# r-barnes/richdem

Hardware: NVIDIA H100
Metric: Priority-Flood fill + D8 flow accumulation throughput (higher is better)
Workload: dtype f32

## Files before the change

richdem_b200/csrc/fill.cu:

```cuda
#include "common.cuh"

#include <chrono>

namespace rdb {

namespace {

#ifndef RDB_TX
#define RDB_TX 64
#endif
#ifndef RDB_TY
#define RDB_TY 64
#endif
#ifndef RDB_FILL_THREADS
#define RDB_FILL_THREADS 128
#endif
#ifndef RDB_FILL_MIN_CTAS
#define RDB_FILL_MIN_CTAS 6
#endif
constexpr int TX = RDB_TX;
constexpr int TY = RDB_TY;
constexpr int BXN = TX / 4;
constexpr int BYN = TY / 4;
constexpr int PADL = 4;
constexpr int SP = TX + 2 * PADL;
constexpr int SROWS = TY + 2;
constexpr int FILL_THREADS = RDB_FILL_THREADS;
constexpr int FILL_MIN_CTAS = RDB_FILL_MIN_CTAS;
static_assert(BYN <= 16 && BXN * BYN <= 256 && TX % 4 == 0 && TY % 4 == 0, "tile shape");
constexpr uint32_t W_TILE_BYTES = SP * SROWS * 4;
constexpr uint32_t Z_TILE_BYTES = TX * TY * 4;

struct RoundCtl {
  int count;
  int take;
};

struct FillDev {
  RoundCtl ctl[3];
  RoundCtl proc[3];
  unsigned long long visits;
  unsigned long long iters;
  unsigned long long block_updates;
  unsigned long long warp_updates;
  unsigned long long idle_visits;
  unsigned long long iter_hist[8];
  int edge_changed;
  int zmin_ord, zmax_ord;
  unsigned long long deferred;
  unsigned long long live_rounds;
  float level, step, step_min, level_max;
  int target, ordered;
  int ndefer[3];
};

struct FillArgs {
  const float *Z;
  int zpitch, zox, zoy, zext;
  const float *coarse;
  int Wc, pool, yoff;
  int *staged;
  float *Wp;
  int pitch;
  int W, H;
  int tilesX, tilesY;
  int *list0, *list1;
  int *stamp;
  int *sides;
  int *keys;
  float level;
  int *plist;
  int use_proc;
  FillDev *dev;
  int round;
  int max_iters;
  int use_tma;
  int profile;
  int *dirty;
};

__device__ __forceinline__ uint32_t smem_u32(const void *p) {
  return (uint32_t)__cvta_generic_to_shared(p);
}
// ... 34 lines not shown

constexpr int NBLK = BXN * BYN;
constexpr int MKP = BXN + 2;
constexpr int NWARP = FILL_THREADS / 32;
constexpr int SEG = ((NBLK + NWARP - 1) / NWARP + 31) / 32 * 32;
enum : int { SIDE_N = 1, SIDE_S = 2, SIDE_W = 4, SIDE_E = 8, SIDE_NW = 16, SIDE_NE = 32, SIDE_SW = 64,
             SIDE_SE = 128, SIDE_FULL = 256 };

__host__ __device__ __forceinline__ int f2ord(float f) {
  int b;
  memcpy(&b, &f, 4);
  return b >= 0 ? b : (b ^ 0x7fffffff);
}
__host__ __device__ __forceinline__ float ord2f(int o) {
  const int b = o >= 0 ? o : (o ^ 0x7fffffff);
  float f;
  memcpy(&f, &b, 4);
  return f;
}
constexpr int ORD_POS_INF = 0x7f800000;

__device__ __forceinline__ void enqueue_tile(const FillArgs &a, RoundCtl *next, int *list_next, int t,
                                             int stampval, int side_bits, int key_ord) {
  atomicOr(&a.sides[(stampval & 1) * a.tilesX * a.tilesY + t], side_bits);
  atomicMin(&a.keys[(stampval & 1) * a.tilesX * a.tilesY + t], key_ord);
  if (atomicExch(&a.stamp[t], stampval) != stampval) {
    const int idx = atomicAdd(&next->count, 1);
    list_next[idx] = t;
  }
}

__device__ __forceinline__ float min3f(float a, float b, float c) { return fminf(fminf(a, b), c); }

template <int STEP, bool TOPO4 = false, bool STAGE = false>
__global__ void __launch_bounds__(FILL_THREADS, FILL_MIN_CTAS)
    fill_sweep_kernel(const __grid_constant__ CUtensorMap mapW, const __grid_constant__ CUtensorMap mapZ,
                      const FillArgs a) {
  __shared__ __align__(128) float sW[SROWS * SP];
  __shared__ __align__(128) float sZ[TY * TX];
  __shared__ __align__(8) unsigned long long mbar;
  __shared__ unsigned char sMark[MKP * (BYN + 2)];
  __shared__ unsigned char sList[2][NWARP][SEG];
  __shared__ __align__(16) int sCnt[2][NWARP];
  __shared__ int sTile;
  __shared__ int sFlags;
  __shared__ int sKey;
  __shared__ int sProf[2];
  __shared__ int sNbDone;

  const int tid = threadIdx.x;
  const int r = a.round;
  RoundCtl *cur = &a.dev->ctl[r % 3];
  RoundCtl *next = &a.dev->ctl[(r + 1) % 3];
  const int *list_cur = (r & 1) ? a.list1 : a.list0;
  int *list_next = (r & 1) ? a.list0 : a.list1;
  const int ntiles = a.tilesX * a.tilesY;
  if (a.use_proc) {
    cur = &a.dev->proc[r % 3];
    list_cur = a.plist;
  }
  const int n = cur->count;

  if (blockIdx.x == 0 && tid == 0) {
    RoundCtl *z = &a.dev->ctl[(r + 2) % 3];
    z->count = 0;
    z->take = 0;
    RoundCtl *zp = &a.dev->proc[(r + 1) % 3];
    zp->count = 0;
    zp->take = 0;
    if (n > 0) {
      atomicAdd(&a.dev->visits, (unsigned long long)n);
      a.dev->live_rounds++;
    }
  }
  if (n == 0) return;

  if (tid == 0) {
    mbar_init(&mbar, 1);
    asm volatile("fence.mbarrier_init.release.cluster;" ::: "memory");
  }
  uint32_t phase = 0;
  const int max_iters = a.max_iters;

  for (;;) {
    if (tid == 0) sTile = atomicAdd(&cur->take, 1);
    for (int k = tid; k < MKP * (BYN + 2); k += FILL_THREADS) sMark[k] = 0;
    __syncthreads();
    const int li = sTile;
    if (li >= n) break;
    const int t = list_cur[li];
    const int tyT = t / a.tilesX, txT = t - tyT * a.tilesX;
    const int x0 = txT * TX, y0 = tyT * TY;

    constexpr bool stage = STAGE;
    if (tid == 0) {
      sFlags = 0;
      sKey = ORD_POS_INF;
      sProf[0] = sProf[1] = 0;
      if (stage) {
        int nb = 0;
        for (int dy = -1; dy <= 1; dy++)
          for (int dx = -1; dx <= 1; dx++) {
            const int ty = tyT + dy, tx = txT + dx;
            if ((dx | dy) && ty >= 0 && ty < a.tilesY && tx >= 0 && tx < a.tilesX &&
                *reinterpret_cast<volatile int *>(&a.staged[ty * a.tilesX + tx]))
              nb |= 1 << ((dy + 1) * 3 + dx + 1);
          }
        __threadfence();
        sNbDone = nb;
      }
    }
    if (a.use_tma) {
      if (tid == 0) {
        fence_proxy_async();
        mbar_arrive_expect_tx(&mbar, (stage ? 0u : W_TILE_BYTES) + Z_TILE_BYTES);
        if (!stage) tma_load_2d(sW, &mapW, x0, y0, &mbar);
        tma_load_2d(sZ, &mapZ, x0 + a.zox, y0 + a.zoy, &mbar);
      }
    } else {
      if (!stage) {
        for (int k = tid; k < SROWS * (SP / 4); k += FILL_THREADS) {
          const int rr = k / (SP / 4), cc = k - rr * (SP / 4);
          reinterpret_cast<float4 *>(sW)[k] =
              __ldcg(reinterpret_cast<const float4 *>(a.Wp + (size_t)(y0 + rr) * a.pitch + x0) + cc);
        }
      }
      const float inf = __int_as_float(0x7f800000);
      for (int k = tid; k < TY * (TX / 4); k += FILL_THREADS) {
        const int rr = k / (TX / 4), cc = k - rr * (TX / 4);
        reinterpret_cast<float4 *>(sZ)[k] =
            a.zext && (y0 + rr >= a.H || x0 + 4 * cc >= a.W)
                ? make_float4(inf, inf, inf, inf)
                : __ldg(reinterpret_cast<const float4 *>(a.Z + (size_t)(y0 + a.zoy + rr) * a.zpitch + x0 + a.zox) + cc);
      }
    }
    int sides = a.sides[(r & 1) * ntiles + t];
    __syncthreads();
    if (tid == 0) {
      a.sides[(r & 1) * ntiles + t] = 0;
      a.keys[(r & 1) * ntiles + t] = ORD_POS_INF;
    }
    if (stage) {
      const float inf = __int_as_float(0x7f800000);
      const int nbdone = sNbDone;
      for (int k = tid; k < SROWS * (SP / 4); k += FILL_THREADS) {
        const int rr = k / (SP / 4), c4 = 4 * (k - rr * (SP / 4));
        const int dy = rr == 0 ? -1 : (rr == SROWS - 1 ? 1 : 0), dx = c4 < PADL ? -1 : (c4 >= PADL + TX ? 1 : 0);
        float4 v4;
        if ((nbdone >> ((dy + 1) * 3 + dx + 1)) & 1) {
          v4 = __ldcg(reinterpret_cast<const float4 *>(a.Wp + (size_t)(y0 + rr) * a.pitch + x0 + c4));
        } else {
          const int y = y0 + rr - 1, xb = x0 + c4 - PADL;
          float v[4] = {inf, inf, inf, inf};
          if (y >= 0 && y < a.H) {
            const float *crow = a.coarse + (size_t)((y + a.yoff) / a.pool) * a.Wc;
            const float *zrow = a.Z + (size_t)(y + a.zoy) * a.zpitch + a.zox;
            const bool brow = y == 0 || y == a.H - 1;
            const float c0 = (a.pool & 3) == 0 && xb >= 0 && xb < a.W ? __ldg(crow + xb / a.pool) : inf;
#pragma unroll
            for (int j = 0; j < 4; j++) {
              const int x = xb + j;
              if (x >= 0 && x < a.W)
                v[j] = brow || x == 0 || x == a.W - 1 ? __ldg(zrow + x) : (a.pool & 3) == 0 ? c0 : __ldg(crow + x / a.pool);
            }
          }
          v4 = make_float4(v[0], v[1], v[2], v[3]);
        }
        *reinterpret_cast<float4 *>(&sW[rr * SP + c4]) = v4;
      }
    }
#include "fill_relax_body.inc"

    if (f) {
      atomicOr(&sFlags, f);
      if (f & 0xFF) atomicMin(&sKey, f2ord(kmin));
    }
    __syncthreads();
    const int fl = sFlags;
    const int rowch = (fl >> 12) & 0xFFFF;
    const int rowout = stage ? (1 << BYN) - 1 : rowch;
    if (rowout) {
      for (int k = tid; k < TY * (TX / 4); k += FILL_THREADS) {
        const int rr = k / (TX / 4), cc = k % (TX / 4);
        if (rowout & (1 << (rr >> 2))) {
          const float4 val = *reinterpret_cast<const float4 *>(&sW[(rr + 1) * SP + PADL + 4 * cc]);
          __stcg(reinterpret_cast<float4 *>(a.Wp + (size_t)(y0 + 1 + rr) * a.pitch + (x0 + PADL)) + cc, val);
        }
      }
    }
    if (stage) {
      __syncthreads();
      if (tid == 0) {
        __threadfence();
        atomicExch(&a.staged[t], 1);
      }
    }
    if (rowch) {
      if (tid < 8) {
        const int sv = r + 1;
        const bool n_ok = tyT > 0, s_ok = tyT < a.tilesY - 1, w_ok = txT > 0, e_ok = txT < a.tilesX - 1;
        int nb = -1, bits = 0;
        switch (tid) {
          case 0: if ((fl & SIDE_N) && n_ok) { nb = t - a.tilesX; bits = SIDE_S; } break;
          case 1: if ((fl & SIDE_S) && s_ok) { nb = t + a.tilesX; bits = SIDE_N; } break;
          case 2: if ((fl & SIDE_W) && w_ok) { nb = t - 1; bits = SIDE_E; } break;
          case 3: if ((fl & SIDE_E) && e_ok) { nb = t + 1; bits = SIDE_W; } break;
          case 4: if ((fl & SIDE_NW) && n_ok && w_ok) { nb = t - a.tilesX - 1; bits = SIDE_SE; } break;
          case 5: if ((fl & SIDE_NE) && n_ok && e_ok) { nb = t - a.tilesX + 1; bits = SIDE_SW; } break;
          case 6: if ((fl & SIDE_SW) && s_ok && w_ok) { nb = t + a.tilesX - 1; bits = SIDE_NE; } break;
          default: if ((fl & SIDE_SE) && s_ok && e_ok) { nb = t + a.tilesX + 1; bits = SIDE_NW; } break;
        }
        if (nb >= 0) enqueue_tile(a, next, list_next, nb, sv, bits, sKey);
        if (tid == 0 && (fl & (3 << 9))) atomicOr(&a.dev->edge_changed, (fl >> 9) & 3);
        if (tid == 0 && a.dirty) a.dirty[t] = 1;
      }
    }
    if (tid == 0) {
      if (again) enqueue_tile(a, next, list_next, t, r + 1, SIDE_FULL, f2ord(-__int_as_float(0x7f800000)));
      atomicAdd(&a.dev->iters, (unsigned long long)iters);
      if (a.profile) {
        if (!rowch) atomicAdd(&a.dev->idle_visits, 1ull);
        atomicAdd(&a.dev->block_updates, (unsigned long long)sProf[0]);
        atomicAdd(&a.dev->warp_updates, (unsigned long long)sProf[1]);
        const int hb = iters <= 1 ? 0 : iters <= 2 ? 1 : iters <= 4 ? 2 : iters <= 8 ? 3 : iters <= 16 ? 4 : iters <= 32 ? 5 : iters <= 64 ? 6 : 7;
        atomicAdd(&a.dev->iter_hist[hb], 1ull);
      }
    }
  }
}

__global__ void __launch_bounds__(256) fill_admit_kernel(const FillArgs a) {
  const int r = a.round;
  const RoundCtl *cur = &a.dev->ctl[r % 3];
  RoundCtl *next = &a.dev->ctl[(r + 1) % 3];
  RoundCtl *proc = &a.dev->proc[r % 3];
  const int *list_cur = (r & 1) ? a.list1 : a.list0;
  int *list_next = (r & 1) ? a.list0 : a.list1;
  const int n = cur->count;
  const int ntiles = a.tilesX * a.tilesY;
  const float level = a.level;
  int nd = 0;
  for (int i = blockIdx.x * blockDim.x + threadIdx.x; i < n; i += gridDim.x * blockDim.x) {
    const int t = list_cur[i];
    const int kord = a.keys[(r & 1) * ntiles + t];
    if (ord2f(kord) <= level) {
      a.plist[atomicAdd(&proc->count, 1)] = t;
    } else {
      int bits = a.sides[(r & 1) * ntiles + t];
      if (bits == 0) bits = SIDE_FULL;
      a.sides[(r & 1) * ntiles + t] = 0;
      a.keys[(r & 1) * ntiles + t] = ORD_POS_INF;
      enqueue_tile(a, next, list_next, t, r + 1, bits, kord);
      nd++;
    }
  }
  for (int o = 16; o > 0; o >>= 1) nd += __shfl_xor_sync(0xffffffffu, nd, o);
  if ((threadIdx.x & 31) == 0 && nd) atomicAdd(&a.dev->ndefer[r % 3], nd);
}

// ... 660 lines not shown
    if (!still_active) first_run = false;
    live_rounds = (int64_t)hd->live_rounds;
    visits_seen = (int64_t)hd->visits;
    iters_seen = (int64_t)hd->iters;
    batch_edge = hd->edge_changed;
    return still_active;
  }
  int64_t iters_seen = 0;

  int run(int64_t max_rounds = 0) {
    Ctx &c = ctx();
    int64_t rounds_this_call = 0;
    int per_sync = (int)(c.params.fill_rounds_per_sync > 0 ? c.params.fill_rounds_per_sync : 16);
    if (max_rounds > 0 && max_rounds < per_sync) per_sync = (int)max_rounds;
    RDB_CK(cudaMemsetAsync(&dev.p->edge_changed, 0, sizeof(int), c.stream));
    for (;;) {
      launch_batch(per_sync);
      collect();
      rounds_this_call += per_sync;
      if (!still_active) break;
      if (max_rounds > 0 && rounds_this_call >= max_rounds) break;
    }
    const FillDev *hd = (const FillDev *)c.pinned;
    c.stats.fill_rounds = live_rounds;
    c.stats.fill_tile_visits = visits_seen;
    c.stats.fill_tile_iters = iters_seen;
    c.stats.fill_tile_cells = TX * TY;
    if (c.params.fill_profile) {
      fprintf(stderr, "[fill profile] deferred=%llu visits=%llu iters=%llu block_updates=%llu (%.1f%% of 256/iter) warp_updates=%llu (%.1f%% of 8/iter) idle_visits=%llu hist(1,2,3-4,5-8,9-16,17-32,33-64,65+)=",
              hd->deferred, hd->visits, hd->iters, hd->block_updates, 100.0 * hd->block_updates / (256.0 * hd->iters + 1),
              hd->warp_updates, 100.0 * hd->warp_updates / (8.0 * hd->iters + 1), hd->idle_visits);
      for (int k = 0; k < 8; k++) fprintf(stderr, "%llu ", hd->iter_hist[k]);
      fprintf(stderr, "\n");
    }
    return batch_edge | (still_active ? 4 : 0);
  }

  void track_dirty() {
    Ctx &c = ctx();
    const size_t nt = (size_t)tilesX * tilesY;
    dirty.alloc(nt);
    RDB_CK(cudaMemsetAsync(dirty.p, 0, nt * sizeof(int), c.stream));
  }
  void clear_dirty() {
    if (dirty.p) RDB_CK(cudaMemsetAsync(dirty.p, 0, (size_t)tilesX * tilesY * sizeof(int), ctx().stream));
  }
  void seed_from_flags(int *d_count = nullptr) {
    Ctx &c = ctx();
    const int nt = tilesX * tilesY;
    FillArgs a = make_args();
    a.round = round;
    fill_seed_flags_kernel<<<(nt + 255) / 256, 256, 0, c.stream>>>(a, tflag.p, nt, d_count);
    RDB_CK(cudaGetLastError());
    count_launch();
  }
  void clear_flags() {
    const size_t nt = (size_t)tilesX * tilesY;
    if (!tflag.p) tflag.alloc(nt);
    RDB_CK(cudaMemsetAsync(tflag.p, 0, nt * sizeof(int), ctx().stream));
  }
  void restrict_into(FillState &cs, int k) {
    Ctx &c = ctx();
    cs.clear_flags();
    const bool selective = dirty.p && TX % k == 0 && TY % k == 0;
    dim3 blk(256), grd((unsigned)((cs.W + 255) / 256), (unsigned)(cs.H < 4096 ? cs.H : 4096));
    fill_restrict_kernel<<<grd, blk, 0, c.stream>>>(Wp.p, pitch, W, H, cs.Wp.p, cs.pitch, cs.W, cs.H, k,
// ... 620 lines not shown
```

richdem_b200/csrc/accum.cu:

```cuda
#include "flowmet.cuh"

#include <cmath>
#include <cooperative_groups.h>
namespace cg = cooperative_groups;

namespace rdb {

namespace {

constexpr uint32_t kDepsMask = 0xFFu;
constexpr uint32_t kSrcFlag = 0x80000000u;
constexpr int kCodeSole = 32;
constexpr int kCodeSource = 64;
constexpr int kLaneChunk = 1024;

template <bool DINF>
__global__ void __launch_bounds__(256) flow_code_kernel(const float *__restrict__ dem, uint8_t *__restrict__ code,
                                                         float *__restrict__ rmaxArr, double *__restrict__ accum,
                                                         int W, int H, float nodata, int ones, int tfilter) {
  const size_t n = (size_t)W * H;
  const size_t i = (size_t)blockIdx.x * blockDim.x + threadIdx.x;
  if (i >= n) return;
  const int y = (int)(i / W), x = (int)(i - (size_t)y * W);
  int cd;
// ... 1402 lines not shown
    frontier[atomicAdd(fcount, 1)] = base_index + x;
  } else {
    row[x] = (left << 56) | val;
  }
}

constexpr int kFaT = 64;
constexpr int kFaCells = kFaT * kFaT;
constexpr int kFaSlots = 4 * kFaT;
constexpr unsigned long long kLkOne = 1ull << 32;

__device__ __forceinline__ int fa_side(int left) { return left < kFaT ? left : kFaT; }

__device__ __forceinline__ int fa_slot_of(int lx, int ly, int tw, int th) {
  if (ly == 0) return lx;
  if (ly == th - 1) return kFaT + lx;
  if (lx == 0) return 2 * kFaT + ly;
  if (lx == tw - 1) return 3 * kFaT + ly;
  return -1;
}

__device__ __forceinline__ bool fa_slot_cell(int s, int tw, int th, int &lx, int &ly) {
  const int k = s & (kFaT - 1), side = s / kFaT;
  if (side < 2) {
    lx = k;
    ly = side == 0 ? 0 : th - 1;
    return k < tw && (side == 0 || th > 1);
  }
  lx = side == 2 ? 0 : tw - 1;
  ly = k;
  return k > 0 && k < th - 1 && (side == 2 || tw > 1);
}

__device__ __forceinline__ void fa_tile_accumulate(const uint8_t *sCode, unsigned long long *sWord, uint16_t *sQueue,
                                                   int *sCount, int tw, int th) {
  const int t = threadIdx.x;
  for (int k = 0; k < kFaCells / 256; k++) {
    const int c = t + 256 * k, lx = c & (kFaT - 1), ly = c / kFaT;
    if (sCode[c] == kCodeNoData) continue;
    unsigned deps = 0;
#pragma unroll
    for (int n = 1; n <= 8; n++) {
      const int x = lx + d8dx(n), y = ly + d8dy(n);
      if (x >= 0 && y >= 0 && x < tw && y < th && (sCode[y * kFaT + x] & 15) == d8_inverse(n)) deps++;
    }
    if (deps) sWord[c] += (unsigned long long)deps << 56;
    else sQueue[atomicAdd(&sCount[0], 1)] = (uint16_t)c;
  }
  __syncthreads();
  const int nsrc = sCount[0];
  int cur = 0;
  unsigned long long acc = 0;
  bool walking = false;
  for (;;) {
    if (!walking) {
      const int i = atomicAdd(&sCount[1], 1);
      if (i >= nsrc) break;
      cur = sQueue[i];
      acc = sWord[cur];
      walking = true;
    }
    const int d = sCode[cur] & 15;
    const int x = (cur & (kFaT - 1)) + d8dx(d), y = cur / kFaT + d8dy(d);
    if (d == 0 || x < 0 || y < 0 || x >= tw || y >= th) {
      walking = false;
      continue;
    }
    const int r = y * kFaT + x;
    const unsigned long long old = atomicAdd(&sWord[r], acc - kPkOne);
    if ((old >> 56) != 1ull) {
      walking = false;
      continue;
    }
    acc = (old & kPkVal) + acc;
    cur = r;
  }
  __syncthreads();
}

constexpr int kFaRootExit = 0x8000, kFaRootEnd = 0x4000;

__global__ void __launch_bounds__(256) fa_tile_codes_kernel(const float *__restrict__ dem, uint8_t *__restrict__ code,
                                                             int *__restrict__ link, unsigned long long *__restrict__ lword,
                                                             unsigned *__restrict__ inflow, int W, int H, float nodata,
                                                             int tiles_x) {
  constexpr int kWin = kFaT + 2;
  static_assert(kFaCells * sizeof(uint16_t) <= kWin * kWin * sizeof(float), "the parent array lives in the DEM window");
  __shared__ __align__(16) float sDem[kWin * kWin];
  __shared__ __align__(16) uint8_t sCode[kFaCells];
  __shared__ unsigned sCount[kFaSlots];
  const int t = threadIdx.x, tile = blockIdx.x;
  sCount[t] = 0;
  const int bx = tile % tiles_x, by = tile / tiles_x;
  const int x0 = bx * kFaT, y0 = by * kFaT;
  const int tw = fa_side(W - x0), th = fa_side(H - y0);
  for (int i = t; i < kWin * kWin; i += 256) {
    const int wy = i / kWin, wx = i - wy * kWin;
    const int gy = y0 - 1 + wy, gx = x0 - 1 + wx;
    sDem[i] = (gy >= 0 && gy < H && gx >= 0 && gx < W) ? __ldg(dem + (size_t)gy * W + gx) : nodata;
  }
  __syncthreads();
  {
    const int lx = t & (kFaT - 1), ly0 = (t / kFaT) * (kFaT / 4);
    float a[3][3];
#pragma unroll
    for (int j = 1; j < 3; j++)
#pragma unroll
      for (int k = 0; k < 3; k++) a[j][k] = sDem[(ly0 + j - 1) * kWin + lx + k];
    for (int j = 0; j < kFaT / 4; j++) {
      const int ly = ly0 + j;
#pragma unroll
      for (int k = 0; k < 3; k++) {
        a[0][k] = a[1][k];
        a[1][k] = a[2][k];
        a[2][k] = sDem[(ly + 2) * kWin + lx + k];
      }
      const float e = a[1][1];
      const int gx = x0 + lx, gy = y0 + ly;
      int cd = 0;
      if (lx >= tw || ly >= th || e == nodata) {
        cd = kCodeNoData;
      } else if (!(gx == 0 || gy == 0 || gx == W - 1 || gy == H - 1)) {
        const float ne[9] = {0.f, a[1][0], a[0][0], a[0][1], a[0][2], a[1][2], a[2][2], a[2][1], a[2][0]};
        float lowest = fminf(e, 3.402823466e+38f);
#pragma unroll
        for (int n = 1; n <= 8; n++) {
          const float v = ne[n];
          if (v < lowest && v != nodata) {
            lowest = v;
            cd = n;
          }
        }
      }
      sCode[ly * kFaT + lx] = (uint8_t)cd;
    }
  }
  __syncthreads();
  reinterpret_cast<uint4 *>(code + (size_t)tile * kFaCells)[t] = reinterpret_cast<const uint4 *>(sCode)[t];
  uint16_t *sPar = reinterpret_cast<uint16_t *>(sDem);
  unsigned live = 0;
#pragma unroll
  for (int k = 0; k < kFaCells / 256; k++) {
    const int c = t + 256 * k, cd = sCode[c], d = cd & 15;
    int p = c | kFaRootEnd;
    if (cd != kCodeNoData && d != 0) {
      const int x = (c & (kFaT - 1)) + d8dx(d), y = c / kFaT + d8dy(d);
      if (x < 0 || y < 0 || x >= tw || y >= th) {
        p = c | kFaRootExit;
      } else {
        p = y * kFaT + x;
        live |= 1u << k;
      }
    }
    sPar[c] = (uint16_t)p;
  }
  while (__syncthreads_or(live)) {
#pragma unroll
    for (int k = 0; k < kFaCells / 256; k++) {
      if (live >> k & 1) {
        const int c = t + 256 * k, q = sPar[sPar[c]];
        sPar[c] = (uint16_t)q;
        if (q & (kFaRootExit | kFaRootEnd)) live &= ~(1u << k);
      }
    }
  }
#pragma unroll
  for (int k = 0; k < kFaCells / 256; k++) {
    const int r = sPar[t + 256 * k];
    if (r & kFaRootExit) atomicAdd(&sCount[fa_slot_of(r & (kFaT - 1), (r & (kFaCells - 1)) / kFaT, tw, th)], 1u);
  }
  __syncthreads();
  const size_t gs = (size_t)tile * kFaSlots + t;
  int lk = -1;
  unsigned long long out = 0;
  int lx, ly;
  if (fa_slot_cell(t, tw, th, lx, ly)) {
    const int c = ly * kFaT + lx, r = sPar[c];
    if (r == (c | kFaRootExit)) {
      const int d = sCode[c] & 15;
      const int gx = x0 + lx + d8dx(d), gy = y0 + ly + d8dy(d), rbx = gx / kFaT, rby = gy / kFaT;
      const int rs = fa_slot_of(gx - rbx * kFaT, gy - rby * kFaT, fa_side(W - rbx * kFaT), fa_side(H - rby * kFaT));
      lk = -2 - ((rby * tiles_x + rbx) * kFaSlots + rs);
      out = kLkOne | sCount[t];
    } else if (r & kFaRootExit) {
      const int e = r & (kFaCells - 1);
      lk = tile * kFaSlots + fa_slot_of(e & (kFaT - 1), e / kFaT, tw, th);
    }
  }
  link[gs] = lk;
  lword[gs] = out;
  inflow[gs] = 0;
}

__device__ __forceinline__ int fa_link_next(const int *link, int r) {
  const int l = link[r];
  return l <= -2 ? r : l;
}

__global__ void __launch_bounds__(256) fa_link_count_kernel(const int *__restrict__ link, unsigned long long *lword,
                                                             int nslots) {
  const int p = blockIdx.x * blockDim.x + threadIdx.x;
  if (p >= nslots) return;
  const int l = link[p];
  if (l > -2) return;
  const int q = fa_link_next(link, -2 - l);
  if (q >= 0) atomicAdd(&lword[q], kLkOne);
}

__global__ void __launch_bounds__(256) fa_link_walk_kernel(const int *__restrict__ link, unsigned long long *lword,
                                                            unsigned *inflow, int nslots) {
  const int p = blockIdx.x * blockDim.x + threadIdx.x;
  if (p >= nslots) return;
  int l = link[p];
  if (l > -2) return;
  const unsigned long long old = atomicAdd(&lword[p], 0ull - kLkOne);
  if ((old >> 32) != 1ull) return;
  unsigned long long acc = old & (kLkOne - 1);
  for (;;) {
    const int r = -2 - l;
    atomicAdd(&inflow[r], (unsigned)acc);
    const int q = fa_link_next(link, r);
    if (q < 0) break;
    const unsigned long long o = atomicAdd(&lword[q], acc - kLkOne);
    if ((o >> 32) != 1ull) break;
    acc = (o & (kLkOne - 1)) + acc;
    l = link[q];
  }
}

__global__ void __launch_bounds__(256) fa_tile_final_kernel(const uint8_t *__restrict__ code,
                                                             const unsigned *__restrict__ inflow, double *__restrict__ accum,
                                                             int W, int H, int tiles_x) {
  __shared__ __align__(16) unsigned long long sWord[kFaCells];
  __shared__ __align__(16) uint8_t sCode[kFaCells];
  __shared__ uint16_t sQueue[kFaCells];
  __shared__ int sCount[2];
  const int t = threadIdx.x, tile = blockIdx.x;
  const int bx = tile % tiles_x, by = tile / tiles_x;
  const int x0 = bx * kFaT, y0 = by * kFaT;
  const int tw = fa_side(W - x0), th = fa_side(H - y0);
  if (t < 2) sCount[t] = 0;
  reinterpret_cast<uint4 *>(sCode)[t] = __ldg(reinterpret_cast<const uint4 *>(code + (size_t)tile * kFaCells) + t);
  for (int c = t; c < kFaCells; c += 256) sWord[c] = 1;
  __syncthreads();
  int lx, ly;
  if (fa_slot_cell(t, tw, th, lx, ly)) sWord[ly * kFaT + lx] += __ldg(inflow + (size_t)tile * kFaSlots + t);
  __syncthreads();
  fa_tile_accumulate(sCode, sWord, sQueue, sCount, tw, th);
  for (int c = t; c < kFaCells; c += 256) {
    const int cx = c & (kFaT - 1), cy = c / kFaT;
    if (cx < tw && cy < th)
      accum[(size_t)(y0 + cy) * W + x0 + cx] = sCode[c] == kCodeNoData ? -1.0 : (double)(sWord[c] & kPkVal);
  }
}

long long fa_tile_slots(int w, int h) {
  return (long long)((w + kFaT - 1) / kFaT) * ((h + kFaT - 1) / kFaT) * kFaSlots;
}

void fa_d8_tiles(const float *d_dem, double *d_accum, int w, int h, float nodata) {
  Ctx &c = ctx();
  const int tiles_x = (w + kFaT - 1) / kFaT;
  const long long nslots = fa_tile_slots(w, h);
  const unsigned ntiles = (unsigned)(nslots / kFaSlots);
  DevBuf<uint8_t> code((size_t)ntiles * kFaCells);
  DevBuf<int> link((size_t)nslots);
  DevBuf<unsigned long long> lword((size_t)nslots);
  DevBuf<unsigned> inflow((size_t)nslots);
  const unsigned sblocks = (unsigned)((nslots + 255) / 256);
  fa_tile_codes_kernel<<<ntiles, 256, 0, c.stream>>>(d_dem, code.p, link.p, lword.p, inflow.p, w, h, nodata, tiles_x);
  fa_link_count_kernel<<<sblocks, 256, 0, c.stream>>>(link.p, lword.p, (int)nslots);
  KernelTimer kt;
  fa_link_walk_kernel<<<sblocks, 256, 0, c.stream>>>(link.p, lword.p, inflow.p, (int)nslots);
  kt.stop_async();
  fa_tile_final_kernel<<<ntiles, 256, 0, c.stream>>>(code.p, inflow.p, d_accum, w, h, tiles_x);
  RDB_CK(cudaGetLastError());
  count_launch(4);
  RDB_CK(cudaStreamSynchronize(c.stream));
  c.stats.ms_main_kernel += kt.ms();
  c.stats.accum_rounds = 1;
}
}

void fa_fused_dev(const float *d_dem, double *d_accum, int w, int h, float nodata, bool ones, bool dinf) {
  Ctx &c = ctx();
  const size_t n = (size_t)w * h;
// ... 865 lines not shown
  FACC_TRY
  state->st.collect_frontier();
  int a = 0, b = 0;
  state->st.run(&a, &b);
  if (sent_top) *sent_top = a;
  if (sent_bottom) *sent_bottom = b;
  FACC_END
}

int rdb200_dev_facc_take_outflow(rdb200_facc_state *state, int32_t which, double *d_sum_row, int32_t *d_cnt_row) {
  FACC_TRY
  state->st.take_outflow(which, d_sum_row, d_cnt_row);
  RDB_CK(cudaStreamSynchronize(rdb::ctx().stream));
  FACC_END
}

int rdb200_dev_facc_apply_inflow(rdb200_facc_state *state, int32_t which, const double *d_sum_row,
                                 const int32_t *d_cnt_row) {
  FACC_TRY
  state->st.apply_inflow(which, d_sum_row, d_cnt_row);
  RDB_CK(cudaStreamSynchronize(rdb::ctx().stream));
  FACC_END
}

int rdb200_dev_facc_finish(rdb200_facc_state *state) {
  FACC_TRY
  if (state) {
    RDB_CK(cudaStreamSynchronize(rdb::ctx().stream));
    delete state;
  }
  FACC_END
}

}
```

richdem_b200/csrc/fill_relax_body.inc:

```
    if (sides == 0) sides = SIDE_FULL;
    const int lane = tid & 31, wrp = tid >> 5;
    {
      int cntw = 0;
#pragma unroll
      for (int q = 0; q < SEG / 32; q++) {
        const int b = wrp * SEG + 32 * q + lane;
        const int bx = b % BXN, by = b / BXN;
        bool on = (sides & SIDE_FULL) != 0;
        on |= (sides & SIDE_N) && by == 0;
        on |= (sides & SIDE_S) && by == BYN - 1;
        on |= (sides & SIDE_W) && bx == 0;
        on |= (sides & SIDE_E) && bx == BXN - 1;
        on |= (sides & SIDE_NW) && b == 0;
        on |= (sides & SIDE_NE) && b == BXN - 1;
        on |= (sides & SIDE_SW) && b == NBLK - BXN;
        on |= (sides & SIDE_SE) && b == NBLK - 1;
        on &= b < NBLK;
        const unsigned bal = __ballot_sync(0xffffffffu, on);
        if (on) sList[0][wrp][cntw + __popc(bal & ((1u << lane) - 1u))] = (unsigned char)b;
        cntw += __popc(bal);
      }
      if (lane == 0) sCnt[0][wrp] = cntw;
    }
    if (a.use_tma) {
      mbar_wait(&mbar, phase);
      phase ^= 1;
      if (a.zext && (x0 + TX > a.W || y0 + TY > a.H)) {
        for (int k = tid; k < TX * TY; k += FILL_THREADS) {
          const int rr = k / TX, cc = k - rr * TX;
          if (y0 + rr >= a.H || x0 + cc >= a.W) sZ[k] = __int_as_float(0x7f800000);
        }
      }
    }
    __syncthreads();

    int f = 0;
    float kmin = __int_as_float(0x7f800000);
    int iters = 0;
    int cl = 0;
    bool again = false;
    int segn[NWARP];
    int nlist = 0;
#pragma unroll
    for (int w2 = 0; w2 < NWARP; w2++) {
      segn[w2] = sCnt[0][w2];
      nlist += segn[w2];
    }
    while (nlist > 0) {
      for (int i = tid; i < nlist; i += FILL_THREADS) {
        int seg = 0, off = i;
#pragma unroll
        for (int w2 = 0; w2 < NWARP - 1; w2++) {
          if (seg == w2 && off >= segn[w2]) {
            off -= segn[w2];
            seg = w2 + 1;
          }
        }
        const int b = sList[cl][seg][off];
        const int bx = b % BXN, by = b / BXN;
        const int srow = 4 * by + 1, scol = 4 * bx + PADL;
        float v[6][6];
        float z[4][4];
        bool at_floor = true;
#pragma unroll
        for (int j = 0; j < 4; j++) {
          const float4 z4 = *reinterpret_cast<const float4 *>(&sZ[(4 * by + j) * TX + 4 * bx]);
          const float4 m4 = *reinterpret_cast<const float4 *>(&sW[(srow + j) * SP + scol]);
// ... 120 lines not shown
```

Measured before the change: 18250.

## Prefetch next tile index and issue TMA early in staged fill sweep

In the staged fill kernel, the next tile index is now claimed from the work queue right after relaxation and before the write-back and enqueue phase, which hides the atomic's latency. TMA loads are issued before the per-tile flag setup rather than after it. Division by the pooling factor uses a shift when the factor is a power of two. The change also adds optional per-phase clock profiling counters. Taking the next tile early changes the order in which tiles are claimed, and it adds a few extra atomics when profiling is on.

```diff
diff --git a/richdem_b200/csrc/fill.cu b/richdem_b200/csrc/fill.cu
--- a/richdem_b200/csrc/fill.cu
+++ b/richdem_b200/csrc/fill.cu
@@ -49,6 +49,7 @@
   int zmin_ord, zmax_ord;
   unsigned long long deferred;
   unsigned long long live_rounds;
+  unsigned long long st_visits, st_iters, st_block_updates, st_hist[8], st_clk[3];
   float level, step, step_min, level_max;
   int target, ordered;
   int ndefer[3];
@@ -149,6 +150,14 @@
 
 __device__ __forceinline__ float min3f(float a, float b, float c) { return fminf(fminf(a, b), c); }
 
+__device__ __forceinline__ unsigned long long prof_clock() {
+#ifdef RDB_EMU
+  return 0;
+#else
+  return clock64();
+#endif
+}
+
 template <int STEP, bool TOPO4 = false, bool STAGE = false>
 __global__ void __launch_bounds__(FILL_THREADS, FILL_MIN_CTAS)
     fill_sweep_kernel(const __grid_constant__ CUtensorMap mapW, const __grid_constant__ CUtensorMap mapZ,
@@ -163,6 +172,7 @@
   __shared__ int sFlags;
   __shared__ int sKey;
   __shared__ int sProf[2];
+  __shared__ unsigned long long sClk;
   __shared__ int sNbDone;
 
   const int tid = threadIdx.x;
@@ -198,18 +208,33 @@
   }
   uint32_t phase = 0;
   const int max_iters = a.max_iters;
-
+  auto prof_phase = [&](int k) {
+    const unsigned long long now = prof_clock();
+    if (k >= 0) atomicAdd(&a.dev->st_clk[k], now - sClk);
+    sClk = now;
+  };
+
+  if (STAGE && tid == 0) sTile = atomicAdd(&cur->take, 1);
   for (;;) {
-    if (tid == 0) sTile = atomicAdd(&cur->take, 1);
+    if (!STAGE && tid == 0) sTile = atomicAdd(&cur->take, 1);
     for (int k = tid; k < MKP * (BYN + 2); k += FILL_THREADS) sMark[k] = 0;
     __syncthreads();
     const int li = sTile;
     if (li >= n) break;
+    if constexpr (STAGE) {
+      if (a.profile && tid == 0) prof_phase(-1);
+    }
     const int t = list_cur[li];
     const int tyT = t / a.tilesX, txT = t - tyT * a.tilesX;
     const int x0 = txT * TX, y0 = tyT * TY;
 
     constexpr bool stage = STAGE;
+    if (a.use_tma && tid == 0) {
+      fence_proxy_async();
+      mbar_arrive_expect_tx(&mbar, (stage ? 0u : W_TILE_BYTES) + Z_TILE_BYTES);
+      if (!stage) tma_load_2d(sW, &mapW, x0, y0, &mbar);
+      tma_load_2d(sZ, &mapZ, x0 + a.zox, y0 + a.zoy, &mbar);
+    }
     if (tid == 0) {
       sFlags = 0;
       sKey = ORD_POS_INF;
@@ -227,14 +252,7 @@
         sNbDone = nb;
       }
     }
-    if (a.use_tma) {
-      if (tid == 0) {
-        fence_proxy_async();
-        mbar_arrive_expect_tx(&mbar, (stage ? 0u : W_TILE_BYTES) + Z_TILE_BYTES);
-        if (!stage) tma_load_2d(sW, &mapW, x0, y0, &mbar);
-        tma_load_2d(sZ, &mapZ, x0 + a.zox, y0 + a.zoy, &mbar);
-      }
-    } else {
+    if (!a.use_tma) {
       if (!stage) {
         for (int k = tid; k < SROWS * (SP / 4); k += FILL_THREADS) {
           const int rr = k / (SP / 4), cc = k - rr * (SP / 4);
@@ -260,6 +278,7 @@
     if (stage) {
       const float inf = __int_as_float(0x7f800000);
       const int nbdone = sNbDone;
+      const int psh = (a.pool & (a.pool - 1)) == 0 ? __ffs(a.pool) - 1 : -1;
       for (int k = tid; k < SROWS * (SP / 4); k += FILL_THREADS) {
         const int rr = k / (SP / 4), c4 = 4 * (k - rr * (SP / 4));
         const int dy = rr == 0 ? -1 : (rr == SROWS - 1 ? 1 : 0), dx = c4 < PADL ? -1 : (c4 >= PADL + TX ? 1 : 0);
@@ -270,15 +289,18 @@
           const int y = y0 + rr - 1, xb = x0 + c4 - PADL;
           float v[4] = {inf, inf, inf, inf};
           if (y >= 0 && y < a.H) {
-            const float *crow = a.coarse + (size_t)((y + a.yoff) / a.pool) * a.Wc;
+            const int cy = psh >= 0 ? (y + a.yoff) >> psh : (y + a.yoff) / a.pool;
+            const float *crow = a.coarse + (size_t)cy * a.Wc;
             const float *zrow = a.Z + (size_t)(y + a.zoy) * a.zpitch + a.zox;
             const bool brow = y == 0 || y == a.H - 1;
-            const float c0 = (a.pool & 3) == 0 && xb >= 0 && xb < a.W ? __ldg(crow + xb / a.pool) : inf;
+            const float c0 = (a.pool & 3) == 0 && xb >= 0 && xb < a.W ? __ldg(crow + (psh >= 0 ? xb >> psh : xb / a.pool)) : inf;
 #pragma unroll
             for (int j = 0; j < 4; j++) {
               const int x = xb + j;
               if (x >= 0 && x < a.W)
-                v[j] = brow || x == 0 || x == a.W - 1 ? __ldg(zrow + x) : (a.pool & 3) == 0 ? c0 : __ldg(crow + x / a.pool);
+                v[j] = brow || x == 0 || x == a.W - 1 ? __ldg(zrow + x)
+                       : (a.pool & 3) == 0            ? c0
+                                                      : __ldg(crow + (psh >= 0 ? x >> psh : x / a.pool));
             }
           }
           v4 = make_float4(v[0], v[1], v[2], v[3]);
@@ -286,7 +308,15 @@
         *reinterpret_cast<float4 *>(&sW[rr * SP + c4]) = v4;
       }
     }
+    if constexpr (STAGE) {
+      if (a.profile && tid == 0) prof_phase(0);
+    }
 #include "fill_relax_body.inc"
+    int next_li = 0;
+    if constexpr (STAGE) {
+      if (a.profile && tid == 0) prof_phase(1);
+      if (tid == 0) next_li = atomicAdd(&cur->take, 1);
+    }
 
     if (f) {
       atomicOr(&sFlags, f);
@@ -341,7 +371,15 @@
         atomicAdd(&a.dev->warp_updates, (unsigned long long)sProf[1]);
         const int hb = iters <= 1 ? 0 : iters <= 2 ? 1 : iters <= 4 ? 2 : iters <= 8 ? 3 : iters <= 16 ? 4 : iters <= 32 ? 5 : iters <= 64 ? 6 : 7;
         atomicAdd(&a.dev->iter_hist[hb], 1ull);
-      }
+        if constexpr (STAGE) {
+          atomicAdd(&a.dev->st_visits, 1ull);
+          atomicAdd(&a.dev->st_iters, (unsigned long long)iters);
+          atomicAdd(&a.dev->st_block_updates, (unsigned long long)sProf[0]);
+          atomicAdd(&a.dev->st_hist[hb], 1ull);
+          prof_phase(2);
+        }
+      }
+      if (STAGE) sTile = next_li;
     }
   }
 }
@@ -1068,6 +1106,16 @@
               hd->warp_updates, 100.0 * hd->warp_updates / (8.0 * hd->iters + 1), hd->idle_visits);
       for (int k = 0; k < 8; k++) fprintf(stderr, "%llu ", hd->iter_hist[k]);
       fprintf(stderr, "\n");
+      if (hd->st_visits) {
+        const double v = (double)hd->st_visits;
+        const double clk = (double)(hd->st_clk[0] + hd->st_clk[1] + hd->st_clk[2]);
+        fprintf(stderr, "[fill profile staged] w=%d h=%d visits=%llu passes/visit=%.2f block_updates/visit=%.1f "
+                        "hist(1,2,3-4,5-8,9-16,17-32,33-64,65+)=",
+                W, H, hd->st_visits, hd->st_iters / v, hd->st_block_updates / v);
+        for (int k = 0; k < 8; k++) fprintf(stderr, "%llu ", hd->st_hist[k]);
+        fprintf(stderr, "clk/visit=%.0f build=%.1f%% relax=%.1f%% write=%.1f%%\n", clk / v, 100.0 * hd->st_clk[0] / clk,
+                100.0 * hd->st_clk[1] / clk, 100.0 * hd->st_clk[2] / clk);
+      }
     }
     return batch_edge | (still_active ? 4 : 0);
   }
```

New measurement: 18380 (median of 6 runs). About the same (+0.7%).

## Pack tile accumulation into 32-bit words with donor counts from code pass

Applied to the files above, without the earlier changes.

The tile-final accumulation now uses 32-bit packed shared words (donor count, direction, local sum) and stores boundary inflow in a separate array that is carried along walks, replacing 64-bit words and the neighbour-scan dependency count. Donor counts are computed once in the codes kernel by atomically adding into the upper nibble of each code byte. Sources are enqueued with a warp prefix scan instead of per-cell atomics. The aim is to cut shared-memory footprint and setup work, at the cost of extra atomics and fences whenever inflow is carried. Optional clock64 phase probes are added behind a macro.

```diff
diff --git a/richdem_b200/csrc/accum.cu b/richdem_b200/csrc/accum.cu
--- a/richdem_b200/csrc/accum.cu
+++ b/richdem_b200/csrc/accum.cu
@@ -1458,47 +1458,70 @@
   return k > 0 && k < th - 1 && (side == 2 || tw > 1);
 }
 
-__device__ __forceinline__ void fa_tile_accumulate(const uint8_t *sCode, unsigned long long *sWord, uint16_t *sQueue,
-                                                   int *sCount, int tw, int th) {
-  const int t = threadIdx.x;
-  for (int k = 0; k < kFaCells / 256; k++) {
-    const int c = t + 256 * k, lx = c & (kFaT - 1), ly = c / kFaT;
-    if (sCode[c] == kCodeNoData) continue;
-    unsigned deps = 0;
-#pragma unroll
-    for (int n = 1; n <= 8; n++) {
-      const int x = lx + d8dx(n), y = ly + d8dy(n);
-      if (x >= 0 && y >= 0 && x < tw && y < th && (sCode[y * kFaT + x] & 15) == d8_inverse(n)) deps++;
-    }
-    if (deps) sWord[c] += (unsigned long long)deps << 56;
-    else sQueue[atomicAdd(&sCount[0], 1)] = (uint16_t)c;
-  }
-  __syncthreads();
-  const int nsrc = sCount[0];
-  int cur = 0;
-  unsigned long long acc = 0;
+#ifdef RDB_FA_PHASE_CLOCKS
+constexpr int kFaPhases = 8;
+__device__ unsigned long long g_fa_phase_clk[2 * kFaPhases];
+#define FA_PHASE_START() long long fa_clk = clock64()
+#define FA_PHASE_END(i)                                                    \
+  do {                                                                     \
+    __syncthreads();                                                       \
+    if (threadIdx.x == 0) {                                                \
+      const long long now = clock64();                                     \
+      atomicAdd(&g_fa_phase_clk[i], (unsigned long long)(now - fa_clk));   \
+      fa_clk = now;                                                        \
+    }                                                                      \
+  } while (0)
+#else
+#define FA_PHASE_START() (void)0
+#define FA_PHASE_END(i) (void)0
+#endif
+
+constexpr unsigned kFwDonor = 1u << 28, kFwCarry = 1u << 24, kFwCarryMask = 15u << 24, kFwSum = (1u << 13) - 1;
+constexpr unsigned kFwNoData = ~0u;
+__device__ __forceinline__ int fw_dir(unsigned w) { return (w >> 20) & 15; }
+
+__device__ __forceinline__ void fa_tile_accumulate(unsigned *sWord, unsigned *sIn, const uint16_t *sQueue, int nsrc,
+                                                   int *sNext, int tw, int th) {
+  int cur = 0, d = 0;
+  unsigned sum = 0, in = 0;
   bool walking = false;
   for (;;) {
     if (!walking) {
-      const int i = atomicAdd(&sCount[1], 1);
+      const int i = atomicAdd(sNext, 1);
       if (i >= nsrc) break;
-      cur = sQueue[i];
-      acc = sWord[cur];
+      const int e = sQueue[i];
+      cur = e & (kFaCells - 1);
+      d = e >> 12;
+      sum = 1;
+      const int cx = cur & (kFaT - 1), cy = cur / kFaT;
+      in = (cx == 0 || cy == 0 || cx == tw - 1 || cy == th - 1) ? sIn[cur] : 0u;
       walking = true;
     }
-    const int d = sCode[cur] & 15;
     const int x = (cur & (kFaT - 1)) + d8dx(d), y = cur / kFaT + d8dy(d);
     if (d == 0 || x < 0 || y < 0 || x >= tw || y >= th) {
       walking = false;
       continue;
     }
     const int r = y * kFaT + x;
-    const unsigned long long old = atomicAdd(&sWord[r], acc - kPkOne);
-    if ((old >> 56) != 1ull) {
+    unsigned add = sum - kFwDonor;
+    if (in) {
+      atomicAdd(&sIn[r], in);
+      __threadfence_block();
+      add += kFwCarry;
+    }
+    const unsigned old = atomicAdd(&sWord[r], add);
+    if ((old >> 28) != 1u) {
       walking = false;
       continue;
     }
-    acc = (old & kPkVal) + acc;
+    sum += old & kFwSum;
+    d = fw_dir(old);
+    if ((old + add) & kFwCarryMask) {
+      __threadfence_block();
+      in = *(volatile unsigned *)&sIn[r];
+    } else {
+      in = 0;
+    }
     cur = r;
   }
   __syncthreads();
@@ -1516,6 +1539,7 @@
   __shared__ __align__(16) uint8_t sCode[kFaCells];
   __shared__ unsigned sCount[kFaSlots];
   const int t = threadIdx.x, tile = blockIdx.x;
+  FA_PHASE_START();
   sCount[t] = 0;
   const int bx = tile % tiles_x, by = tile / tiles_x;
   const int x0 = bx * kFaT, y0 = by * kFaT;
@@ -1526,6 +1550,7 @@
     sDem[i] = (gy >= 0 && gy < H && gx >= 0 && gx < W) ? __ldg(dem + (size_t)gy * W + gx) : nodata;
   }
   __syncthreads();
+  FA_PHASE_END(0);
   {
     const int lx = t & (kFaT - 1), ly0 = (t / kFaT) * (kFaT / 4);
     float a[3][3];
@@ -1562,7 +1587,7 @@
     }
   }
   __syncthreads();
-  reinterpret_cast<uint4 *>(code + (size_t)tile * kFaCells)[t] = reinterpret_cast<const uint4 *>(sCode)[t];
+  FA_PHASE_END(1);
   uint16_t *sPar = reinterpret_cast<uint16_t *>(sDem);
   unsigned live = 0;
 #pragma unroll
@@ -1576,10 +1601,12 @@
       } else {
         p = y * kFaT + x;
         live |= 1u << k;
+        atomicAdd(reinterpret_cast<unsigned *>(sCode) + (p >> 2), 16u << (8 * (p & 3)));
       }
     }
     sPar[c] = (uint16_t)p;
   }
+  FA_PHASE_END(2);
   while (__syncthreads_or(live)) {
 #pragma unroll
     for (int k = 0; k < kFaCells / 256; k++) {
@@ -1590,6 +1617,8 @@
       }
     }
   }
+  FA_PHASE_END(3);
+  reinterpret_cast<uint4 *>(code + (size_t)tile * kFaCells)[t] = reinterpret_cast<const uint4 *>(sCode)[t];
 #pragma unroll
   for (int k = 0; k < kFaCells / 256; k++) {
     const int r = sPar[t + 256 * k];
@@ -1616,6 +1645,7 @@
   link[gs] = lk;
   lword[gs] = out;
   inflow[gs] = 0;
+  FA_PHASE_END(4);
 }
 
 __device__ __forceinline__ int fa_link_next(const int *link, int r) {
@@ -1657,27 +1687,73 @@
 __global__ void __launch_bounds__(256) fa_tile_final_kernel(const uint8_t *__restrict__ code,
                                                              const unsigned *__restrict__ inflow, double *__restrict__ accum,
                                                              int W, int H, int tiles_x) {
-  __shared__ __align__(16) unsigned long long sWord[kFaCells];
-  __shared__ __align__(16) uint8_t sCode[kFaCells];
+  __shared__ __align__(16) unsigned sWord[kFaCells];
+  __shared__ __align__(16) unsigned sIn[kFaCells];
   __shared__ uint16_t sQueue[kFaCells];
   __shared__ int sCount[2];
   const int t = threadIdx.x, tile = blockIdx.x;
+  FA_PHASE_START();
   const int bx = tile % tiles_x, by = tile / tiles_x;
   const int x0 = bx * kFaT, y0 = by * kFaT;
   const int tw = fa_side(W - x0), th = fa_side(H - y0);
   if (t < 2) sCount[t] = 0;
-  reinterpret_cast<uint4 *>(sCode)[t] = __ldg(reinterpret_cast<const uint4 *>(code + (size_t)tile * kFaCells) + t);
-  for (int c = t; c < kFaCells; c += 256) sWord[c] = 1;
+  int lx, ly;
+  const bool slot = fa_slot_cell(t, tw, th, lx, ly);
+  const unsigned seed = slot ? __ldg(inflow + (size_t)tile * kFaSlots + t) : 0u;
+  const uint4 cv = __ldg(reinterpret_cast<const uint4 *>(code + (size_t)tile * kFaCells) + t);
   __syncthreads();
-  int lx, ly;
-  if (fa_slot_cell(t, tw, th, lx, ly)) sWord[ly * kFaT + lx] += __ldg(inflow + (size_t)tile * kFaSlots + t);
+  const unsigned cw[4] = {cv.x, cv.y, cv.z, cv.w};
+  unsigned src = 0;
+#pragma unroll
+  for (int j = 0; j < 4; j++) {
+    unsigned w[4];
+#pragma unroll
+    for (int b = 0; b < 4; b++) {
+      const unsigned cd = cw[j] >> (8 * b) & 0xFF;
+      w[b] = cd == kCodeNoData ? kFwNoData : (cd >> 4) * kFwDonor | (cd & 15) << 20 | 1u;
+      const int c = 16 * t + 4 * j + b, d = cd & 15;
+      const int x = (c & (kFaT - 1)) + d8dx(d), y = c / kFaT + d8dy(d);
+      if (cd < 16 && d != 0 && x >= 0 && y >= 0 && x < tw && y < th) src |= 1u << (4 * j + b);
+    }
+    reinterpret_cast<uint4 *>(sWord)[4 * t + j] = make_uint4(w[0], w[1], w[2], w[3]);
+    reinterpret_cast<uint4 *>(sIn)[t + 256 * j] = make_uint4(0, 0, 0, 0);
+  }
+  {
+    const int lane = t & 31, n = __popc(src);
+    int incl = n;
+#pragma unroll
+    for (int o = 1; o < 32; o <<= 1) {
+      const int v = __shfl_up_sync(0xffffffffu, incl, o);
+      if (lane >= o) incl += v;
+    }
+    int base = 0;
+    if (lane == 31) base = atomicAdd(&sCount[0], incl);
+    int pos = __shfl_sync(0xffffffffu, base, 31) + incl - n;
+    for (unsigned m = src; m; m &= m - 1) {
+      const int k = __ffs(m) - 1;
+      const unsigned four = k < 8 ? (k < 4 ? cv.x : cv.y) : (k < 12 ? cv.z : cv.w);
+      sQueue[pos++] = (uint16_t)((16 * t + k) | (four >> (8 * (k & 3)) & 15) << 12);
+    }
+  }
   __syncthreads();
-  fa_tile_accumulate(sCode, sWord, sQueue, sCount, tw, th);
+  FA_PHASE_END(8);
+  if (seed) {
+    const int c = ly * kFaT + lx;
+    sIn[c] = seed;
+    sWord[c] += kFwCarry;
+  }
+  __syncthreads();
+  FA_PHASE_END(9);
+  fa_tile_accumulate(sWord, sIn, sQueue, sCount[0], &sCount[1], tw, th);
+  FA_PHASE_END(10);
   for (int c = t; c < kFaCells; c += 256) {
     const int cx = c & (kFaT - 1), cy = c / kFaT;
+    const unsigned w = sWord[c];
     if (cx < tw && cy < th)
-      accum[(size_t)(y0 + cy) * W + x0 + cx] = sCode[c] == kCodeNoData ? -1.0 : (double)(sWord[c] & kPkVal);
-  }
+      accum[(size_t)(y0 + cy) * W + x0 + cx] =
+          w == kFwNoData ? -1.0 : (double)((unsigned long long)(w & kFwSum) + sIn[c]);
+  }
+  FA_PHASE_END(11);
 }
 
 long long fa_tile_slots(int w, int h) {
@@ -2609,4 +2685,16 @@
   FACC_END
 }
 
-}
+#ifdef RDB_FA_PHASE_CLOCKS
+RDB200_API int rdb200_fa_phase_clocks(unsigned long long *out) {
+  FACC_TRY
+  rdb::ensure_init();
+  RDB_CK(cudaStreamSynchronize(rdb::ctx().stream));
+  RDB_CK(cudaMemcpyFromSymbol(out, rdb::g_fa_phase_clk, sizeof(rdb::g_fa_phase_clk)));
+  const unsigned long long zero[2 * rdb::kFaPhases] = {};
+  RDB_CK(cudaMemcpyToSymbol(rdb::g_fa_phase_clk, zero, sizeof(zero)));
+  FACC_END
+}
+#endif
+
+}
```

Measured after the change: 16760 before, 17760 after, median of 6. 1.06x the previous value.

## Add warp-parallel vertical drain sweeps before block relaxation in staged fill

Applied to the files above, without the earlier changes.

Before the block-list relaxation in STAGE kernels, adds a pass where each warp sweeps its column strip down (or up) the 64x64 tile, propagating water levels through rows using shuffles, and records changed rows, sides and the edge minimum key. This is meant to carry long-range drainage across the tile in one pass instead of through many block-local iterations. Separately, the staging loop is rewritten with a fixed per-thread column and incrementally updated coarse row/column indices, which removes per-element integer divisions by pool. The sweep adds work and two syncs on every staged tile, and it only turns on for the 64x64/128-thread configuration.

```diff
diff --git a/richdem_b200/csrc/fill.cu b/richdem_b200/csrc/fill.cu
--- a/richdem_b200/csrc/fill.cu
+++ b/richdem_b200/csrc/fill.cu
@@ -149,6 +149,68 @@
 
 __device__ __forceinline__ float min3f(float a, float b, float c) { return fminf(fminf(a, b), c); }
 
+constexpr bool DRAIN_SWEEPS = TX == 64 && TY == 64 && FILL_THREADS == 128;
+
+template <bool TOPO4>
+__device__ __forceinline__ void fill_drain_sweeps(float *sW, const float *sZ, int y0, int H, int *sFlags, int *sKey) {
+  const unsigned FULL = 0xffffffffu;
+  const int tid = threadIdx.x, lane = tid & 31, wrp = tid >> 5;
+  const int x = 32 * (wrp & 1) + lane;
+  const bool down = wrp < 2;
+  const int dy = down ? 1 : -1;
+  const bool ecol = x < 4 || x >= TX - 4;
+  unsigned long long rows = 0;
+  float kmin = __int_as_float(0x7f800000);
+  int y = down ? 0 : TY - 1;
+  float p = sW[(y - dy + 1) * SP + PADL + x];
+#pragma unroll 1
+  for (int half = 0; half < 2; half++) {
+#pragma unroll 8
+    for (int s = 0; s < TY / 2; s++, y += dy) {
+      const float zz = sZ[y * TX + x];
+      float *cell = &sW[(y + 1) * SP + PADL + x];
+      const float w = *cell;
+      float m = p;
+      if (!TOPO4) {
+        float pl = __shfl_up_sync(FULL, p, 1), pr = __shfl_down_sync(FULL, p, 1);
+        const float *prow = &sW[(y - dy + 1) * SP + PADL + x];
+        if (lane == 0) pl = prow[-1];
+        if (lane == 31) pr = prow[1];
+        m = min3f(pl, p, pr);
+      }
+      const float nw = fminf(w, fmaxf(zz, m));
+      p = w;
+      if (nw < w) {
+        *cell = nw;
+        p = nw;
+        rows |= 1ull << y;
+        if (ecol || y < 4 || y >= TY - 4) kmin = fminf(kmin, nw);
+      }
+    }
+    __syncthreads();
+  }
+  int f = 0;
+#pragma unroll
+  for (int by = 0; by < BYN; by++)
+    if ((rows >> (4 * by)) & 0xFull) f |= 1 << (12 + by);
+  if (rows & 1ull) f |= SIDE_N;
+  if (rows >> (TY - 1)) f |= SIDE_S;
+  if (x == 0 && rows) f |= SIDE_W | (rows & 1ull ? SIDE_NW : 0) | (rows >> (TY - 1) ? SIDE_SW : 0);
+  if (x == TX - 1 && rows) f |= SIDE_E | (rows & 1ull ? SIDE_NE : 0) | (rows >> (TY - 1) ? SIDE_SE : 0);
+  const int j1 = 1 - y0, j2 = (H - 2) - y0;
+  if (j1 >= 0 && j1 < TY && ((rows >> j1) & 1ull)) f |= 1 << 9;
+  if (j2 >= 0 && j2 < TY && ((rows >> j2) & 1ull)) f |= 1 << 10;
+#pragma unroll
+  for (int o = 16; o > 0; o >>= 1) {
+    f |= __shfl_xor_sync(FULL, f, o);
+    kmin = fminf(kmin, __shfl_xor_sync(FULL, kmin, o));
+  }
+  if (lane == 0 && f) {
+    atomicOr(sFlags, f);
+    if (f & 0xFF) atomicMin(sKey, f2ord(kmin));
+  }
+}
+
 template <int STEP, bool TOPO4 = false, bool STAGE = false>
 __global__ void __launch_bounds__(FILL_THREADS, FILL_MIN_CTAS)
     fill_sweep_kernel(const __grid_constant__ CUtensorMap mapW, const __grid_constant__ CUtensorMap mapZ,
@@ -260,30 +322,52 @@
     if (stage) {
       const float inf = __int_as_float(0x7f800000);
       const int nbdone = sNbDone;
-      for (int k = tid; k < SROWS * (SP / 4); k += FILL_THREADS) {
-        const int rr = k / (SP / 4), c4 = 4 * (k - rr * (SP / 4));
-        const int dy = rr == 0 ? -1 : (rr == SROWS - 1 ? 1 : 0), dx = c4 < PADL ? -1 : (c4 >= PADL + TX ? 1 : 0);
-        float4 v4;
-        if ((nbdone >> ((dy + 1) * 3 + dx + 1)) & 1) {
-          v4 = __ldcg(reinterpret_cast<const float4 *>(a.Wp + (size_t)(y0 + rr) * a.pitch + x0 + c4));
-        } else {
-          const int y = y0 + rr - 1, xb = x0 + c4 - PADL;
-          float v[4] = {inf, inf, inf, inf};
-          if (y >= 0 && y < a.H) {
-            const float *crow = a.coarse + (size_t)((y + a.yoff) / a.pool) * a.Wc;
-            const float *zrow = a.Z + (size_t)(y + a.zoy) * a.zpitch + a.zox;
-            const bool brow = y == 0 || y == a.H - 1;
-            const float c0 = (a.pool & 3) == 0 && xb >= 0 && xb < a.W ? __ldg(crow + xb / a.pool) : inf;
+      constexpr int C4N = SP / 4, RSTEP = FILL_THREADS / C4N;
+      static_assert(RSTEP >= 1, "a CTA covers one row of the window");
+      if (tid < RSTEP * C4N) {
+        const int c4 = 4 * (tid % C4N);
+        int rr = tid / C4N;
+        const int dx = c4 < PADL ? -1 : (c4 >= PADL + TX ? 1 : 0);
+        const int xb = x0 + c4 - PADL;
+        const int cx = xb >= 0 ? xb / a.pool : 0, rx = xb - cx * a.pool;
+        const int yy = y0 + rr - 1 + a.yoff;
+        int cy = (yy + a.pool) / a.pool - 1, ry = yy - cy * a.pool;
+        const int dq = RSTEP / a.pool, dr = RSTEP - dq * a.pool;
+        for (; rr < SROWS; rr += RSTEP) {
+          const int dy = rr == 0 ? -1 : (rr == SROWS - 1 ? 1 : 0);
+          float4 v4;
+          if ((nbdone >> ((dy + 1) * 3 + dx + 1)) & 1) {
+            v4 = __ldcg(reinterpret_cast<const float4 *>(a.Wp + (size_t)(y0 + rr) * a.pitch + x0 + c4));
+          } else {
+            const int y = y0 + rr - 1;
+            float v[4] = {inf, inf, inf, inf};
+            if (y >= 0 && y < a.H) {
+              const float *crow = a.coarse + (size_t)cy * a.Wc;
+              const float *zrow = a.Z + (size_t)(y + a.zoy) * a.zpitch + a.zox;
+              const bool brow = y == 0 || y == a.H - 1;
+              const float c0 = (a.pool & 3) == 0 && xb >= 0 && xb < a.W ? __ldg(crow + cx) : inf;
+              int cc = cx, rc = rx;
 #pragma unroll
-            for (int j = 0; j < 4; j++) {
-              const int x = xb + j;
-              if (x >= 0 && x < a.W)
-                v[j] = brow || x == 0 || x == a.W - 1 ? __ldg(zrow + x) : (a.pool & 3) == 0 ? c0 : __ldg(crow + x / a.pool);
+              for (int j = 0; j < 4; j++) {
+                const int x = xb + j;
+                if (j > 0 && ++rc == a.pool) {
+                  rc = 0;
+                  cc++;
+                }
+                if (x >= 0 && x < a.W)
+                  v[j] = brow || x == 0 || x == a.W - 1 ? __ldg(zrow + x) : (a.pool & 3) == 0 ? c0 : __ldg(crow + cc);
+              }
             }
+            v4 = make_float4(v[0], v[1], v[2], v[3]);
           }
-          v4 = make_float4(v[0], v[1], v[2], v[3]);
+          *reinterpret_cast<float4 *>(&sW[rr * SP + c4]) = v4;
+          cy += dq;
+          ry += dr;
+          if (ry >= a.pool) {
+            ry -= a.pool;
+            cy++;
+          }
         }
-        *reinterpret_cast<float4 *>(&sW[rr * SP + c4]) = v4;
       }
     }
 #include "fill_relax_body.inc"
diff --git a/richdem_b200/csrc/fill_relax_body.inc b/richdem_b200/csrc/fill_relax_body.inc
--- a/richdem_b200/csrc/fill_relax_body.inc
+++ b/richdem_b200/csrc/fill_relax_body.inc
@@ -33,6 +33,7 @@
       }
     }
     __syncthreads();
+    if constexpr (STAGE && DRAIN_SWEEPS) fill_drain_sweeps<TOPO4>(sW, sZ, y0, a.H, &sFlags, &sKey);
 
     int f = 0;
     float kmin = __int_as_float(0x7f800000);
```

New measurement: 17880 before, 18550 after (median of 6 runs). 3.8% higher.
